# ryought/dbgphmm

Hardware: AMD Instinct MI355X
Metric: read-bases/sec through forward+backward P(R|X) (higher is better)
Workload: dtype f64; 1 GPU; cfg3: synthetic 100 kb diploid genome (1% divergence), 20x HiFi reads (p=0.001, L=1000), k=40 DBG; sparse-adaptive forward+backward+posteriors (generate_mappings); n_nodes=131694, n_edges=132357, reads_rank0=4026, bases_rank0=4000713, total_bases=4000713, spin_up_steps=12

## Files before the change

### dbgphmm_amd/csrc/api.cpp

```cpp
#include <chrono>
#include <cstdlib>
#include <cmath>
#include <cstring>

#include "phmm_internal.h"

namespace phmm {

static thread_local std::string g_error;
static thread_local hipStream_t g_stream = nullptr;
static thread_local uint64_t g_ws_limit = 0;
static thread_local CallStats g_stats;
static thread_local bool g_timing = false;

void set_error(const std::string &msg) { g_error = msg; }
int fail(int code, const std::string &msg) {
    g_error = msg;
    return code;
}
hipStream_t current_stream() { return g_stream; }
int &workset_index() {
    static thread_local int idx = 0;
    return idx;
}
ThreadContext capture_thread_context() {
    ThreadContext c{g_ws_limit, g_timing, 0};
    (void)hipGetDevice(&c.device);
    return c;
}
void adopt_thread_context(const ThreadContext &c, hipStream_t stream, int workset) {
    (void)hipSetDevice(c.device);
    g_ws_limit = c.ws_limit;
    g_timing = c.timing;
    g_stream = stream;
    g_stats = CallStats();
    workset_index() = workset;
}
static thread_local ShareInfo g_share;
CallStats &stats() { return g_stats; }
ShareInfo &share_info() { return g_share; }
bool timing_enabled() { return g_timing; }

uint64_t workspace_limit() {
    if (g_ws_limit) return g_ws_limit;
    size_t fr = 0, tot = 0;
    if (hipMemGetInfo(&fr, &tot) != hipSuccess) return (uint64_t)16 << 30;
    return (uint64_t)(0.8 * (double)fr);
}

static Knobs g_knobs;
const Knobs &knobs() { return g_knobs; }
void refresh_knobs() {
    auto flag = [](const char *n) {
        const char *e = std::getenv(n);
        return e != nullptr && e[0] != '\0' && !(e[0] == '0' && e[1] == '\0');
    };
    auto num = [](const char *n, int dflt) {
        const char *e = std::getenv(n);
        return e ? std::atoi(e) : dflt;
    };
    Knobs k;
    k.trace = flag("PHMM_TRACE");
    k.no_lean = flag("PHMM_NO_LEAN");
    k.no_wide_class = flag("PHMM_NO_WIDE_CLASS");
    k.no_packed = flag("PHMM_NO_PACKED");
    k.packed_cpl = num("PHMM_PACKED_CPL", 0);
    k.no_exact_hinted = flag("PHMM_NO_EXACT_HINTED");
    k.no_exact_dense = flag("PHMM_NO_EXACT_DENSE");
    k.no_wide_hinted = flag("PHMM_NO_WIDE_HINTED");
    k.wide_hinted = flag("PHMM_WIDE_HINTED") && !k.no_wide_hinted;
    k.no_wide_list_bwd = flag("PHMM_NO_WIDE_LIST_BWD");
    k.wide_edge_bwd = flag("PHMM_WIDE_EDGE_BWD");
    k.wide_states_bwd = flag("PHMM_WIDE_STATES_BWD");
    k.wide_bwd_t = num("PHMM_WIDE_BWD_T", 0);
    if (k.wide_bwd_t != 128 && k.wide_bwd_t != 448) k.wide_bwd_t = 0;
    k.wide_hinted_cpb = num("PHMM_WIDE_HINTED_CPB", 0);
    if (k.wide_hinted_cpb != 1 && k.wide_hinted_cpb != 2 && k.wide_hinted_cpb != 4) k.wide_hinted_cpb = 0;
    k.no_side_worker = flag("PHMM_NO_SIDE_WORKER");
    k.no_wide_handover = flag("PHMM_NO_WIDE_HANDOVER");
    k.workers = std::max(1, std::min(MAX_WORKERS, num("PHMM_WORKERS", 1)));
    k.warm_cols = num("PHMM_WARM_COLS", 0);
    k.chunk_groups = std::max(0, num("PHMM_CHUNK_GROUPS", 0));
    k.no_keep_all = flag("PHMM_NO_KEEP_ALL");
    k.pipeline_min_groups = std::max(1, num("PHMM_PIPELINE_MIN_GROUPS", 8));
    k.no_runmax = flag("PHMM_NO_RUNMAX");
    k.force_radix = flag("PHMM_FORCE_RADIX");
    k.no_bwd_skip = flag("PHMM_NO_BWD_SKIP");
    k.serial_emit = flag("PHMM_SERIAL_EMIT");
    k.emit_high_priority = flag("PHMM_EMIT_HIGH_PRIORITY");
    k.no_dma = flag("PHMM_NO_DMA");
    k.bwd_dma = flag("PHMM_BWD_DMA");
    k.dense_streams = num("PHMM_DENSE_STREAMS", 0);
    k.dense_w = num("PHMM_DENSE_W", 0);
    k.dense_npt = num("PHMM_DENSE_NPT", 0);
    if (const char *e = std::getenv("PHMM_MEM_FRACTION")) k.mem_fraction = std::min(0.97, std::max(0.1, std::atof(e)));
    k.share_prefix = num("PHMM_SHARE_PREFIX", -1);
    if (k.share_prefix < 0 || k.share_prefix > 6) k.share_prefix = -1;
    g_knobs = k;
}

void trace(const char *tag) {
    if (!g_knobs.trace) return;
    static thread_local std::chrono::steady_clock::time_point last = std::chrono::steady_clock::now();
    (void)hipStreamSynchronize(g_stream);
    const auto now = std::chrono::steady_clock::now();
    static const auto t0 = std::chrono::steady_clock::now();
    std::fprintf(stderr, "[phmm trace] w%d @%9.2f %-28s %8.2f ms\n", workset_index(),
                 std::chrono::duration<double, std::milli>(now - t0).count(), tag,
                 std::chrono::duration<double, std::milli>(now - last).count());
    last = now;
}

uint64_t table_budget(const DevicePool &pool, uint64_t reserve) {
    if (g_ws_limit) return g_ws_limit;
    size_t fr = 0, tot = 0;
    if (hipMemGetInfo(&fr, &tot) != hipSuccess) return (uint64_t)16 << 30;
    const double frac = g_knobs.mem_fraction > 0.0 ? g_knobs.mem_fraction : 0.9;
    const double b = frac * (double)(fr + pool.owned_table_bytes()) - (double)reserve;
    return (uint64_t)std::max(b, 64.0 * 1024 * 1024);
}
uint64_t planned_budget(const DevicePool &pool) {
    if (g_ws_limit) return g_ws_limit;
    size_t fr = 0, tot = 0;
    if (hipMemGetInfo(&fr, &tot) != hipSuccess) return (uint64_t)16 << 30;
    const double frac = g_knobs.mem_fraction > 0.0 ? g_knobs.mem_fraction : 0.95;
    return (uint64_t)(frac * (double)(fr + pool.owned_bytes()));
}

static std::mutex g_pool_mu;
static DevicePool *g_pools[64] = {};
DevicePool &device_pool() {
    int dev = 0;
    (void)hipGetDevice(&dev);
    if (dev < 0 || dev >= 64) PHMM_THROW(PHMM_ENODEVICE, "device index out of range");
    std::lock_guard<std::mutex> lk(g_pool_mu);
    if (!g_pools[dev]) {
        g_pools[dev] = new DevicePool();
        g_pools[dev]->device = dev;
    }
    return *g_pools[dev];
}
void DevicePool::recycle(DevBuf &b) {
    if (!b.p) return;
    std::lock_guard<std::mutex> lk(spare_mu);
    if (b.bytes < ((size_t)1 << 20) || b.bytes > SPARE_BYTES) {
        b.release();
        return;
    }
    while (!spare.empty() && (spare.size() >= SPARE_MAX || spare_total + b.bytes > SPARE_BYTES)) {
        (void)hipFree(spare.front().first);
        spare_total -= spare.front().second;
        spare.erase(spare.begin());
    }
    spare_total += b.bytes;
    const size_t n = b.bytes;
    spare.emplace_back(b.detach(), n);
}
void DevicePool::take(DevBuf &b, size_t n) {
    if (n <= b.bytes) return;
    {
        std::lock_guard<std::mutex> lk(spare_mu);
        int best = -1;
        for (int i = 0; i < (int)spare.size(); i++)
            if (spare[i].second >= n && spare[i].second <= 2 * n &&
                (best < 0 || spare[i].second < spare[best].second))
                best = i;
        if (best >= 0) {
            b.adopt(spare[best].first, spare[best].second);
            spare_total -= spare[best].second;
            spare.erase(spare.begin() + best);
// ... 892 lines not shown
```

### dbgphmm_amd/csrc/dense.hip

```cpp
#include <algorithm>
#include <cmath>
#include <cstring>
#include <numeric>
#include <type_traits>

#include "dense_internal.h"
#include "lds_dma.h"
#include "prefix_share.h"

#ifndef PHMM_FWD_PF
#define PHMM_FWD_PF 2
#endif
#ifndef PHMM_BWD_PF
#define PHMM_BWD_PF 1
#endif
#ifndef PHMM_SMALLW_WAVES
#define PHMM_SMALLW_WAVES 3
#endif

namespace phmm {


__device__ __forceinline__ int xcd_block(int b, int nblk8) {
    int per = nblk8 >> 3;
// ... 352 lines not shown
}

template <int W>
__global__ void __launch_bounds__(BLOCK) fwd_finish(const DenseArgs a) {
    __shared__ double lds[(BLOCK / 64) * 64];
    const int g = blockIdx.x;
    const int col = blockIdx.y;
    constexpr int ROWS = BLOCK / W;
    const int r = threadIdx.x % W, row = threadIdx.x / W;
    const int len = a.len[g * W + r];
    const size_t ecols = a.eall ? (size_t)a.Lc : 1;
    double s = 0.0;
    const bool live = a.eall ? col < len : len > 0;
    if (live)
        for (int b = row; b < a.nblk; b += ROWS)
            s += a.epart[(((size_t)g * ecols + col) * a.nblk8 + b) * W + r];
    const double tot = block_reduce_rows<W>(s, OpAdd(), lds);
    if (threadIdx.x < W && live) {
        const int E = a.FE[((size_t)g * (a.Lc + 1) + (a.eall ? col + 1 : len)) * W + r];
        const double lp = log(a.lp.p_end * tot) + (double)E * LN2;
        if (a.eall) a.logE[((size_t)g * a.Lc + col) * W + r] = lp;
        if (!a.eall || col == len - 1) a.logPf[g * W + r] = lp;
    }
}

__device__ __forceinline__ double dev_logadd(double x, double y) {
    const double hi = x >= y ? x : y, lo = x >= y ? y : x;
    if (lo == -INFINITY) return hi;
    return hi + log1p(exp(lo - hi));
}

template <int W>
__device__ __forceinline__ void bwd_chain(const DenseArgs &a, int g, int p, double *lds) {
    constexpr int ROWS = BLOCK / W;
    const int r = threadIdx.x % W, row = threadIdx.x / W;
    const int len = a.len[g * W + r];
    const bool live = p < len && (!a.bstart || p <= (a.bstart[g * W + r] & ~(1 << 30)));
    double s1 = 0.0, s2 = 0.0;
    if (live) {
        const double *bp = a.bpart + ((size_t)(p & 1) * a.ng + g) * a.nblk8 * W * 2;
        for (int b = row; b < a.nblk; b += ROWS) {
            s1 += bp[((size_t)b * W + r) * 2 + 0];
            s2 += bp[((size_t)b * W + r) * 2 + 1];
        }
    }
    const double t1 = block_reduce_rows<W>(s1, OpAdd(), lds);
    const double t2 = block_reduce_rows<W>(s2, OpAdd(), lds);
    if (threadIdx.x < W && live) {
        const size_t ix = ((size_t)g * (a.Lc + 1) + p) * W + r;
        const double E = (double)a.BE[ix] * LN2;
        const double ibn = (p + 1 < len) ? a.logibB[ix + W] : -INFINITY;
        const double lr = log(a.lp.p_random);
        a.logmbB[ix] = dev_logadd(log(t1) + E, log(a.lp.p_MI) + lr + ibn);
        a.logibB[ix] = dev_logadd(log(t2) + E, log(a.lp.p_II) + lr + ibn);
    }
}

static constexpr int BDMA_DEPTH = 3;
static constexpr int BDMA_SLOT = 5 * 64;
template <int W, bool DMA, bool VF = false>
__global__ void __launch_bounds__(BLOCK, (W == 64 ? 4 : PHMM_SMALLW_WAVES)) bwd_step(const DenseArgs a, const int pos) {
    static_assert(!VF || (W == 64 && !DMA), "the virtual-table loads go through the register ring of bwd_step<64>");
    __shared__ double lds[(BLOCK / 64) * 64];
    constexpr bool DMA_ = DMA && W == 64;
    __shared__ double ring[DMA_ ? (BLOCK / 64) * BDMA_DEPTH * BDMA_SLOT : 1];
    const int g = blockIdx.y + a.g_off;
    const int lb = xcd_block(blockIdx.x, a.nblk8);
    constexpr int ROWS = BLOCK / W;
    const int r = threadIdx.x % W;
    const int row = threadIdx.x / W;
    const int len = a.len[g * W + r];
    const int braw = a.bstart ? a.bstart[g * W + r] : len - 1;
    const bool sparse_tail = (braw & (1 << 30)) != 0;
    const int bstart = braw & ~(1 << 30);
    const bool live = pos < len && pos <= bstart;
    const bool first = live && pos == len - 1;
    const LinParams &lp = a.lp;
    const size_t NW = (size_t)a.N * W;

    if (lb == 0 && pos + 1 < a.Lc) bwd_chain<W>(a, g, pos + 1, lds);

    bool compute = true;
    int hull_first = 0, hull_top = a.npt - 1;
    if (W == 64 && a.skA) {
        compute = false;
        const int rho = __builtin_amdgcn_readfirstlane(lb * ROWS + row);
        if (__any(live) && rho < a.nrun) {
            const size_t gs = (size_t)g * a.nseg, gr = (size_t)g * a.nrun, par = (size_t)a.ng * a.nrun;
            const uint32_t *hh = a.skH + gs;
            const uint8_t *an = a.skA + (size_t)((pos + 1) & 1) * par + gr;
            const int sh = pos + 1 < 31 ? pos + 1 : 31;
            const int sprs = segs_per_run_log2(a.npt), spr = 1 << sprs;
            const unsigned anyfirst = __any(first) ? 1u : 0u;
            const int ls = threadIdx.x & 63;
            const int sg = rho * spr + ls;
            unsigned f = 0;
            if (ls < spr && sg < a.nseg) {
                f = (hh[sg] >> sh) | (((unsigned)an[rho] >> ls) & 1u) | anyfirst;
                const uint32_t o0 = a.rs_off[sg], o1 = a.rs_off[sg + 1];
                for (uint32_t q = o0; q < o1 && !f; q++) {
                    const uint32_t t = a.rs[q];
                    f = (hh[t] >> sh) | (((unsigned)an[t >> sprs] >> (t & (uint32_t)(spr - 1))) & 1u);
                }
            }
            const unsigned mask = (unsigned)__builtin_amdgcn_readfirstlane((int)(unsigned)__ballot(f != 0));
            const int kb = rho * a.npt;
            compute = seg_hull(mask, a.sseg, a.npt - 1 < a.N - 1 - kb ? a.npt - 1 : a.N - 1 - kb, &hull_first, &hull_top);
            if (ls == 0) a.skA[(size_t)(pos & 1) * par + gr + rho] = (uint8_t)mask;
        }
    }
    if (!__syncthreads_or(live && (compute || lb == 0))) {
        if (threadIdx.x < W && lb < a.nblk) {
            double *bp = a.bpart + ((size_t)(pos & 1) * a.ng + g) * a.nblk8 * W * 2;
            bp[((size_t)lb * W + r) * 2 + 0] = 0.0;
            bp[((size_t)lb * W + r) * 2 + 1] = 0.0;
        }
        if (a.want_map && a.Prun) a.Prun[((size_t)g * a.nblk8 + lb) * BLOCK + threadIdx.x] = 0.0;
        return;
    }

    int Epos = 0;
    double sc = 1.0;
    if (live && !first) {
        const unsigned long long cm = a.cmaxB[((size_t)g * a.Lc + (pos + 1)) * W + r];
        const int e = exp_of_bits(cm);
        sc = pow2(-e);
        Epos = a.BE[((size_t)g * (a.Lc + 1) + (pos + 1)) * W + r] + e;
    }
    const uint8_t x = live ? a.bases[((size_t)g * a.Lc + pos) * W + r] : (uint8_t)0;
    const int cn = a.bcols == 2 ? ((pos + 1) & 1) : (pos + 1 < a.Lc ? pos + 1 : 0);
    const int cc = a.bcols == 2 ? (pos & 1) : pos;
    const double *nm = a.Bm + ((size_t)g * a.bcols + cn) * NW;
    const double *ni = a.Bi + ((size_t)g * a.bcols + cn) * NW;
    double *om = a.Bm + ((size_t)g * a.bcols + cc) * NW;
    double *oi = a.Bi + ((size_t)g * a.bcols + cc) * NW;
    double *od = a.Bd ? a.Bd + ((size_t)g * a.bcols + cc) * NW : nullptr;

    double wgt = 0.0, wgt2 = 0.0;
    const double *fm = nullptr, *fi = nullptr, *fd = nullptr, *gm = nullptr, *gi = nullptr, *gd = nullptr;
    const bool want_post = a.want_freq || a.want_map;
    if (want_post && live) {
        const double lpf = a.logPf[g * W + r];
        if (lpf > -INFINITY) {
            if (pos >= 1) {
                const int fe = a.FE[((size_t)g * (a.Lc + 1) + (pos - 1)) * W + r];
                wgt = exp((double)(fe + Epos) * LN2 - lpf);
            }
            if (first && !sparse_tail) {
                const int fe = a.FE[((size_t)g * (a.Lc + 1) + pos) * W + r];
                wgt2 = exp((double)fe * LN2 - lpf) * lp.p_end;
            }
        }
    }
    if (want_post) {
        const size_t cprev = ((size_t)g * a.Lc + (pos > 0 ? pos - 1 : 0)) * NW;
        const size_t ccur = ((size_t)g * a.Lc + pos) * NW;
        fm = a.Fm + cprev; fi = a.Fi + cprev; fd = a.Fd + cprev;
        gm = a.Fm + ccur; gi = a.Fi + ccur; gd = a.Fd + ccur;
    }
    int rf = r;
    if (VF && want_post) {
        const uint32_t v = share_lane_of_column(a.vlane[g * W + r], pos - 1);
        const size_t vc = ((size_t)(v / SHARE_W) * a.vLc + (pos - 1)) * NW;
        fm = a.vFm + vc; fi = a.vFi + vc; fd = a.vFd + vc;
        rf = (int)(v % SHARE_W);
    }

    double vmax = 0.0, s1 = 0.0, s2 = 0.0, pmx = 0.0, pmx2 = 0.0;
    double *Pa = a.want_map ? a.Pa + (size_t)g * NW : nullptr;
    double *Pb = a.want_map ? a.Pb + (size_t)g * NW : nullptr;
    if (lb < a.nblk && compute) {
        constexpr int H = CHAIN_HOPS;
        const int kbase = lb * (a.npt * ROWS) + row * a.npt + hull_first;
        double E1 = 0.0, E2 = 0.0, E3 = 0.0, E4 = 0.0, E5 = 0.0, Q1 = 0.0, Q2 = 0.0, Q3 = 0.0, Q4 = 0.0, Q5 = 0.0, TE = 0.0;
        int nvalid = 0;
        constexpr int PFB = DMA_ ? BDMA_DEPTH : PHMM_BWD_PF;
        double nx_m[PFB], nx_i[PFB], nx_fm[PFB], nx_fi[PFB], nx_fd[PFB];
        const double *lfm = want_post ? fm : nm, *lfi = want_post ? fi : nm, *lfd = want_post ? fd : nm;
        const int jtop = hull_top < a.N - 1 - kbase ? hull_top : a.N - 1 - kbase;
        const int l64 = threadIdx.x & 63;
        const double *srcA = (l64 < 32 ? nm : ni) + 2 * (l64 & 31);
        const double *srcB = (l64 < 32 ? lfm : lfi) + 2 * (l64 & 31);
        const double *srcC = lfd + 2 * (l64 & 31);
        const uint32_t ring_base =
            DMA_ ? (uint32_t)__builtin_amdgcn_readfirstlane(
                       (int)(uint32_t)(uintptr_t)&ring[(threadIdx.x >> 6) * BDMA_DEPTH * BDMA_SLOT])
                 : 0u;
// ... 970 lines not shown
```

### dbgphmm_amd/csrc/dense_internal.h

```cpp
#pragma once

#include <vector>

#include "phmm_internal.h"
#include "seg_hull.h"

namespace phmm {

static constexpr double LN2 = 0.693147180559945309417232121458;
static constexpr int BLOCK = 256;

struct DenseArgs {
    int N, ng, Lc, nblk, npt;
    int g_off;
    const NodeRec *nodes;
    const uint8_t *emis;
    const double *init, *dinit, *tdinit;
    const uint32_t *fc_off;
    const FwdEntry *fc;
    const uint32_t *bc_off;
    const BwdEntry *bc;
    const uint32_t *fh_off, *bh_off;
    const HopEntry *fh, *bh;
    int hop_mode;
    LinParams lp;
    const double *logib;
    const uint8_t *bases;
    const int *len;
    double *Fm, *Fi, *Fd;
    int *FE;
    unsigned long long *cmaxF;
    double *epart;
    int eall;
    double *logPf;
    double *logE;
    double *Bm, *Bi, *Bd;
    int bcols;
    int *BE;
    unsigned long long *cmaxB;
    double *bpart;
    double *logmbB, *logibB;
    double *accg;
    int want_freq;
    int nblk8;
    unsigned long long *tmaxF;
    const int *bstart;
    int want_map;
    double *Pa, *Pb;
    double *Prun;
    unsigned long long *pmax;
    const int *wf_sw;
    const uint8_t *wf_mode;
    int *wf_sub;
    int *wf_cnt;
    uint32_t *wf_node;
    double *wf_tot;
    double wf_ratio;
    double wf_ub_a, wf_ub_b;
    const uint32_t *rs_off = nullptr, *rs = nullptr;
    uint32_t *skH = nullptr;
    uint8_t *skA = nullptr;
    int nrun = 0, nseg = 0, sseg = 1;
    unsigned long long *skcells = nullptr;
    const double *vFm = nullptr, *vFi = nullptr, *vFd = nullptr;
    const uint32_t *vlane = nullptr;
    int vLc = 0, vJ = 0;
};
static constexpr int WF_CAP = 1024;


struct Plan {
    int W, ng_total, npt, nblk, nblk8;
    std::vector<uint32_t> order;
};

Plan make_plan(const phmm_model *m, const phmm_reads *reads, int forced_w);
Plan make_plan_ids(const phmm_model *m, const phmm_reads *reads, const std::vector<uint32_t> &ids);
void layout(DenseArgs &a, int W, bool full_b, void *tables, void *misc, size_t &tb, size_t &mb,
            bool backward_only = false);
void fill_model_args(DenseArgs &a, const phmm_model *m);
void host_logib(const phmm_model *m, size_t n, std::vector<double> &out);
void launch_fwd_step(int W, const DenseArgs &a, int pos);
void launch_fwd_finish(int W, const DenseArgs &a);
void launch_bwd_step(int W, const DenseArgs &a, int pos);
void launch_bwd_finish(int W, const DenseArgs &a);

struct ExactTables {
    double *f_m, *f_i, *f_d, *f_scal, *b_m, *b_i, *b_d, *b_scal;
};
void exact_dense_reads(phmm_model *m, const uint8_t *bases, const uint64_t *off, const std::vector<uint32_t> &ids, double *lf,
                       double *lb, double *freq_dev, const ExactTables *tabs, double *edge_freq_dev = nullptr,
                       double *init_freq_dev = nullptr);
bool certify_dense(int N, int len, double log2P, const int *FE, const double *log2maxF, const int *BE, const double *log2maxB,
                   double log2_p_end);
bool certify_dense_cells(int N, int len, const int *E, const double *log2max, bool backward);

}
```

### dbgphmm_amd/csrc/mapping_flow.hip

```cpp
#include <algorithm>
#include <cmath>
#include <cstring>
#include <memory>

#include <hipcub/hipcub.hpp>

#include "sparse_dyn.h"
#include "lean_bwd_kernel.h"
#include "wide_bwd_kernel.h"

namespace phmm {

static constexpr int KMAX = PHMM_MAX_ACTIVE_NODES;

template <int CAP> struct FRec {
    double m[CAP], i[CAP], d[CAP];
    uint32_t id[CAP];
    int n, na, E;
};

template <int CAP> __device__ bool load_record(const RecPool &p, uint64_t pos_index, FRec<CAP> &f) {
    const uint64_t o1 = p.off[pos_index];
    if (o1 == 0) return false;
    const uint8_t *rec = p.base + (o1 - 8);
// ... 821 lines not shown
            const double u = bval[q];
            rank += (u > v) || (u == v && bid[q] < id);
        }
        if (rank < need && nabove + rank < KMAX) {
            ids[nabove + rank] = id;
            val[nabove + rank] = v;
        }
    }
    __syncthreads();
    const int tot = nabove + (nb < need ? nb : need);
    return tot < KMAX ? tot : KMAX;
}

__global__ void __launch_bounds__(BLOCK) emit_dense_map(const DenseMapArgs ma, const int pos, const int lanes) {
    __shared__ uint32_t ids[KMAX];
    __shared__ double val[KMAX];
    __shared__ uint16_t order[KMAX];
    const DenseArgs &a = ma.d;
    if ((int)blockIdx.x >= ma.wl_count[1]) return;
    const uint32_t item = ma.wl_big[blockIdx.x];
    const int gi = (int)(item % (uint32_t)lanes), which = (int)(item / (uint32_t)lanes);
    const int len = a.len[gi];
    if (len == 0) return;
    const int braw = a.bstart[gi];
    const bool sparse_tail = (braw & (1 << 30)) != 0;
    const int bstart = braw & ~(1 << 30);
    const bool live = pos < len && pos <= bstart;
    const bool mine = which == 0 ? (live && pos >= 1) : (live && pos == len - 1 && !sparse_tail);
    if (!mine) return;
    int *cnt = which == 0 ? ma.cntA : ma.cntB;
    const int c = cnt[gi];
    const int g = gi / ma.W, r = gi % ma.W;
    const int mi = which == 0 ? pos : len;
    int n = c < KMAX ? c : KMAX;
    if (c > KMAX) {
        const double *P = (which == 0 ? a.Pa : a.Pb) + (size_t)g * a.N * ma.W + r;
        const double vmax = __longlong_as_double((long long)a.pmax[((size_t)g * (a.Lc + 1) + mi) * ma.W + r]);
        n = block_top_from_column(P, ma.W, a.N, vmax * ma.ratio_lin, vmax, ids, val, ma.force_radix != 0);
    } else {
        const uint32_t *cn = (which == 0 ? ma.candA_node : ma.candB_node) + (size_t)gi * KMAX;
        const double *cv = (which == 0 ? ma.candA_val : ma.candB_val) + (size_t)gi * KMAX;
        for (int j = threadIdx.x; j < n; j += BLOCK) {
            ids[j] = cn[j];
            val[j] = cv[j];
        }
    }
    __syncthreads();
    if (ma.topk > 0 && n < ma.topk && n < a.N && threadIdx.x == 0) {
        const int want = ma.topk < a.N ? ma.topk : a.N;
        const int n0 = n;
        for (uint32_t k = 0; n < want && k < (uint32_t)a.N; k++) {
            bool present = false;
            for (int j = 0; j < n0; j++) present |= ids[j] == k;
            if (!present) {
                ids[n] = k;
                val[n] = 0.0;
                n++;
            }
        }
        cnt[gi] = -n;
    }
    __syncthreads();
    if (cnt[gi] < 0) n = -cnt[gi];
    __syncthreads();
    if (threadIdx.x >= 64) return;
    const uint64_t pidx = ma.lane_pos0[gi] + (uint64_t)(mi - 1);
    if (!emit_mapping<KMAX>(ma.mpool, pidx, ids, val, n, ma.ratio_lin, true, order, ma.topk,
                            (long long)ma.eoff[item])) {
        if (threadIdx.x == 0) atomicOr(&ma.err[gi], SP_ERR_POOL);
    }
    if (threadIdx.x == 0) cnt[gi] = 0;
}

__global__ void __launch_bounds__(BLOCK) gather_logb(const double *logmbB, int Lc, int W, int lanes, double *out) {
    const int gi = blockIdx.x * BLOCK + threadIdx.x;
    if (gi < lanes) out[gi] = logmbB[(size_t)(gi / W) * (Lc + 1) * W + gi % W];
}

__global__ void __launch_bounds__(BLOCK) merge_logp(const uint32_t *lanes, int n, const double *src, double *dst) {
    const int j = blockIdx.x * BLOCK + threadIdx.x;
    if (j < n) dst[lanes[j]] = src[lanes[j]];
}

namespace {
template <int W> void launch_post_collect(const DenseMapArgs &ma, int pos) {
    hipLaunchKernelGGL(post_collect<W>, dim3(ma.d.nblk, ma.d.ng), dim3(BLOCK), 0, current_stream(), ma, pos);
}
void launch_post_collect_w(int W, const DenseMapArgs &ma, int pos) {
    switch (W) {
    case 1: launch_post_collect<1>(ma, pos); break;
    case 2: launch_post_collect<2>(ma, pos); break;
    case 4: launch_post_collect<4>(ma, pos); break;
    case 8: launch_post_collect<8>(ma, pos); break;
    case 16: launch_post_collect<16>(ma, pos); break;
    case 32: launch_post_collect<32>(ma, pos); break;
    case 64: launch_post_collect<64>(ma, pos); break;
    default: PHMM_THROW(PHMM_EINTERNAL, "bad read-group width");
    }
}
}

void mapping_backward_chunk(MapChunk &mc, const std::vector<uint32_t> &sparse_lanes, MappingSink *sink,
                            const Plan &plan, int g0, uint64_t R) {
    hipStream_t s = current_stream();
    CallStats &st = stats();
    phmm_model *m = mc.m;
    const int W = mc.W, lanes = mc.lanes;
    const std::vector<int> &hl = *mc.hl, &hsw = *mc.hsw;
    const std::vector<uint64_t> &lp0 = *mc.lane_pos0;
    const size_t NW = (size_t)m->N * W;

    std::vector<int> hb(lanes, 0);
    std::vector<uint64_t> gp0(lanes + 1, 0);
    int pos_max = -1;
    for (int gi = 0; gi < lanes; gi++) {
        const size_t slot = (size_t)g0 * W + gi;
        if (hl[gi] == 0 || slot >= R) {
            hb[gi] = -1;
            continue;
        }
        gp0[gi] = sink->reads->off[plan.order[slot]];
        if (hsw[gi] < hl[gi]) hb[gi] = hsw[gi] | (1 << 30);
        else hb[gi] = hl[gi] - 1;
        pos_max = std::max(pos_max, hb[gi] & ~(1 << 30));
    }
    DevBuf &ctl = m->wset().aux[3], &pbuf = m->wset().aux[4];
    const bool skip = W == 64 && !knobs().no_bwd_skip && pos_max >= 0;
    const int sseg = seg_size(mc.a.npt);
    const RunSucc *rsucc = skip ? &model_run_successors(m, sseg) : nullptr;
    const size_t sk_nrun = ((size_t)m->N + mc.a.npt - 1) / mc.a.npt;
    size_t cb = 0;
    auto carve = [&](size_t bytes) {
        cb = (cb + 255) / 256 * 256;
        size_t o = cb;
        cb += bytes;
        return o;
    };
    const size_t o_bs = carve(sizeof(int) * lanes), o_ca = carve(sizeof(int) * lanes * 2), o_cb = carve(sizeof(int) * lanes * 2),
                 o_err = carve(sizeof(uint32_t) * lanes), o_cells = carve(sizeof(unsigned long long)), o_lanes = carve(sizeof(uint32_t) * std::max<size_t>(sparse_lanes.size(), 1)),
                 o_lp0 = carve(sizeof(uint64_t) * (lanes + 1)), o_gp0 = carve(sizeof(uint64_t) * (lanes + 1)),
                 o_stop = carve(sizeof(int) * lanes),
                 o_skh = carve(skip ? sizeof(uint32_t) * (size_t)mc.a.ng * rsucc->nseg : 0), o_ska = carve(skip ? 2 * (size_t)mc.a.ng * sk_nrun : 0),
                 o_bn = carve(sizeof(uint32_t) * (size_t)lanes * KMAX * 2), o_bv = carve(sizeof(double) * (size_t)lanes * KMAX * 2),
                 o_an = carve(sizeof(uint32_t) * (size_t)lanes * KMAX * 2), o_av = carve(sizeof(double) * (size_t)lanes * KMAX * 2),
                 o_hand = carve(sizeof(BHandoff) * (size_t)lanes), o_eoff = carve(sizeof(unsigned long long) * 2 * (size_t)lanes),
                 o_wls = carve(sizeof(uint32_t) * 2 * (size_t)lanes), o_wlb = carve(sizeof(uint32_t) * 2 * (size_t)lanes),
                 o_wlc = carve(sizeof(int) * 2), o_lb = carve(sizeof(double) * (size_t)lanes);
    ctl.reserve(cb);
    char *cp = (char *)ctl.p;
    const size_t prun_n = (size_t)mc.ngc * mc.a.nblk8 * BLOCK;
    bool need_pb = false;
    for (int gi = 0; gi < lanes; gi++) need_pb |= hb[gi] >= 0 && !(hb[gi] & (1 << 30));
    pbuf.reserve(((need_pb ? 3 : 2) * (size_t)mc.ngc * NW + prun_n) * sizeof(double));
    unsigned long long top_before = 0;
    HIP_CHECK(hipMemcpyAsync(&top_before, sink->mp.top, sizeof(top_before), hipMemcpyDeviceToHost, s));
    HIP_CHECK(hipStreamSynchronize(s));

    for (int attempt = 0;; attempt++) {
        HIP_CHECK(hipMemsetAsync(cp, 0, o_bn, s));
        HIP_CHECK(hipMemcpyAsync(cp + o_bs, hb.data(), sizeof(int) * lanes, hipMemcpyHostToDevice, s));
        HIP_CHECK(hipMemcpyAsync(cp + o_lp0, lp0.data(), sizeof(uint64_t) * (lanes + 1), hipMemcpyHostToDevice, s));
        HIP_CHECK(hipMemcpyAsync(cp + o_gp0, gp0.data(), sizeof(uint64_t) * (lanes + 1), hipMemcpyHostToDevice, s));
        if (!sparse_lanes.empty())
            HIP_CHECK(hipMemcpyAsync(cp + o_lanes, sparse_lanes.data(), sizeof(uint32_t) * sparse_lanes.size(),
                                     hipMemcpyHostToDevice, s));
        const RecPool mp = sink->mp;

        DenseArgs a = mc.a;
        a.want_freq = 0;
        a.want_map = 1;
        a.bstart = (const int *)(cp + o_bs);
        a.Pa = pbuf.as<double>();
        a.Pb = need_pb ? pbuf.as<double>() + 2 * (size_t)mc.ngc * NW : pbuf.as<double>();
        a.Prun = knobs().no_runmax ? nullptr : pbuf.as<double>() + (need_pb ? 3 : 2) * (size_t)mc.ngc * NW;
        const bool st_on = W == 64 && mc.main_plan;
        if (skip) {
            a.rs_off = rsucc->off.as<uint32_t>();
            a.rs = rsucc->ent.as<uint32_t>();
            a.nseg = (int)rsucc->nseg;
            a.sseg = sseg;
            a.nrun = (int)sk_nrun;
            a.skH = (uint32_t *)(cp + o_skh);
            a.skA = (uint8_t *)(cp + o_ska);
            a.skcells = st_on ? (unsigned long long *)(cp + o_cells) : nullptr;
            HIP_CHECK(hipMemsetAsync(pbuf.p, 0, sizeof(double) * 2 * (size_t)mc.ngc * NW, s));
        }
        HIP_CHECK(hipMemsetAsync(a.cmaxB, 0, sizeof(unsigned long long) * (size_t)a.ng * a.Lc * W, s));
        HIP_CHECK(hipMemsetAsync(a.pmax, 0, sizeof(unsigned long long) * (size_t)a.ng * (a.Lc + 1) * W, s));
        HIP_CHECK(hipMemsetAsync(a.BE, 0, sizeof(int) * (size_t)a.ng * (a.Lc + 1) * W, s));
        HIP_CHECK(hipMemsetAsync(a.Bm, 0, sizeof(double) * (size_t)a.ng * a.bcols * NW, s));
        HIP_CHECK(hipMemsetAsync(a.Bi, 0, sizeof(double) * (size_t)a.ng * a.bcols * NW, s));

        if (!sparse_lanes.empty()) {
            hipLaunchKernelGGL(merge_logp, dim3((unsigned)((sparse_lanes.size() + BLOCK - 1) / BLOCK)), dim3(BLOCK), 0, s,
                               (const uint32_t *)(cp + o_lanes), (int)sparse_lanes.size(), mc.d_logp_sparse, a.logPf);
            SparseBwdArgs ba{};
            ba.M = mc.fa_M;
            ba.d = a;
            ba.W = W;
            ba.Lb = mc.Lfull;
            ba.sw = mc.d_sw;
            ba.bases = mc.d_bases_full;
            ba.fpool = mc.fpool;
            ba.mpool = mp;
            ba.lane_pos0 = (const uint64_t *)(cp + o_lp0);
            ba.map_pos0 = (const uint64_t *)(cp + o_gp0);
            ba.lanes = (const uint32_t *)(cp + o_lanes);
            ba.ratio_lin = mc.ratio_lin;
            ba.topk = mc.topk;
            ba.err = (uint32_t *)(cp + o_err);
            ba.stop = (int *)(cp + o_stop);
            ba.hand = (BHandoff *)(cp + o_hand);
            std::vector<uint32_t> todo;
            std::vector<int> hstop(lanes);
            std::vector<uint32_t> herr2(lanes);
            const bool lean_ok =
                mc.topk == 0 && m->dev.max_degree <= (uint32_t)ADJ_DEG && !knobs().no_lean;
            const bool wide_ok = lean_ok && !knobs().no_wide_class;
            const int slice = mc.Lfull > 6144 ? 4096 : 0;
            std::vector<uint32_t> cont = sparse_lanes, big, fresh;
            bool first = true, any_err = false;
            int bursts = 0;
            auto launch = [&](int kind, int mode, int steps, const std::vector<uint32_t> &who) {
                HIP_CHECK(hipMemcpyAsync(cp + o_lanes, who.data(), sizeof(uint32_t) * who.size(), hipMemcpyHostToDevice, s));
                ba.mode = mode;
                ba.max_steps = steps;
                if (kind == 0 && lean_ok)
                    hipLaunchKernelGGL(lean_backward_kernel, dim3((unsigned)who.size()), dim3(64), 0, s, ba);
                else if (kind == 0)
                    hipLaunchKernelGGL((sparse_backward_kernel<64>), dim3((unsigned)who.size()), dim3(64), 0, s, ba);
                else if (wide_ok)
                    hipLaunchKernelGGL(wide_backward_kernel<false>, dim3((unsigned)who.size()), dim3(WBK_T), 0, s, ba);
                else
                    hipLaunchKernelGGL((sparse_backward_kernel<KMAX>), dim3((unsigned)who.size()), dim3(64), 0, s, ba);
                HIP_CHECK(hipGetLastError());
                st.launches[3]++;
                HIP_CHECK(hipMemcpyAsync(hstop.data(), ba.stop, sizeof(int) * lanes, hipMemcpyDeviceToHost, s));
                HIP_CHECK(hipMemcpyAsync(herr2.data(), ba.err, sizeof(uint32_t) * lanes, hipMemcpyDeviceToHost, s));
                HIP_CHECK(hipStreamSynchronize(s));
            };
            for (int turn = 0; turn < 100000 && !any_err && (!cont.empty() || !big.empty() || !fresh.empty()); turn++) {
                std::vector<uint32_t> ncont;
                if (!cont.empty()) {
                    launch(0, first ? 0 : 1, lean_ok ? slice : 0, cont);
                    for (uint32_t gi : cont) {
                        if (herr2[gi] & ~SP_STOP_SLICE) any_err = true;
                        else if (hstop[gi] == hsw[gi]) continue;
                        else if (herr2[gi] & SP_STOP_SLICE) ncont.push_back(gi);
                        else if (first && hstop[gi] == hl[gi]) fresh.push_back(gi);
                        else big.push_back(gi);
                    }
                    first = false;
                }
                if (any_err) break;
                const int burst = slice > 0 ? (64 << std::min(bursts, 5)) : 0;
                for (int pass = 0; pass < 2 && !any_err; pass++) {
                    std::vector<uint32_t> &who = pass == 0 ? fresh : big;
                    if (who.empty()) continue;
                    launch(1, pass == 0 ? 0 : 1, burst, who);
                    for (uint32_t gi : who) {
                        if (herr2[gi] & ~SP_STOP_SLICE) any_err = true;
                        else if (hstop[gi] != hsw[gi]) ncont.push_back(gi);
                    }
                    who.clear();
                    bursts++;
                }
                cont.swap(ncont);
            }
            todo = cont;
            todo.insert(todo.end(), big.begin(), big.end());
            todo.insert(todo.end(), fresh.begin(), fresh.end());
            if (!todo.empty()) {
                bool perr = false;
                HIP_CHECK(hipMemcpy(herr2.data(), ba.err, sizeof(uint32_t) * lanes, hipMemcpyDeviceToHost));
                for (uint32_t gi : sparse_lanes) perr |= (herr2[gi] & ~SP_STOP_SLICE) != 0;
                if (!perr) PHMM_THROW(PHMM_EINTERNAL, "sparse backward did not finish");
            }
        }
        trace("  sparse backward");
        DenseMapArgs ma{};
        ma.d = a;
        ma.W = W;
        ma.mpool = mp;
        ma.lane_pos0 = (const uint64_t *)(cp + o_gp0);
        ma.ratio_lin = mc.ratio_lin;
        ma.topk = mc.topk;
        ma.err = (uint32_t *)(cp + o_err);
        ma.eoff = (unsigned long long *)(cp + o_eoff);
        ma.wl_small = (uint32_t *)(cp + o_wls);
        ma.wl_big = (uint32_t *)(cp + o_wlb);
        ma.wl_count = (int *)(cp + o_wlc);
        std::vector<int> live_at((size_t)pos_max + 2, 0);
        for (int gi = 0; gi < lanes; gi++)
            if (hb[gi] >= 0) live_at[(size_t)(hb[gi] & ~(1 << 30))]++;
        for (int p = pos_max - 1; p >= 0; p--) live_at[(size_t)p] += live_at[(size_t)p + 1];
        ma.force_radix = knobs().force_radix ? 1 : 0;
        LaunchTimer lt(timing_enabled() && st_on);
        std::unique_lock<std::mutex> dense_lock;
        if (mc.dense_token) dense_lock = std::unique_lock<std::mutex>(*mc.dense_token);
        const int wi = workset_index();
        if (!m->pool->cstream[wi]) {
            int least = 0, greatest = 0;
            HIP_CHECK(hipDeviceGetStreamPriorityRange(&least, &greatest));
            HIP_CHECK(hipStreamCreateWithPriority(&m->pool->cstream[wi], hipStreamNonBlocking, knobs().emit_high_priority ? greatest : least));
        }
        for (auto &e : m->pool->cevent[wi])
            if (!e) HIP_CHECK(hipEventCreateWithFlags(&e, hipEventDisableTiming));
        hipStream_t s2 = knobs().serial_emit ? s : m->pool->cstream[wi];
        hipEvent_t *ev_col = &m->pool->cevent[wi][0], *ev_emit = &m->pool->cevent[wi][2];
        bool emitted[2] = {false, false};
        for (int pos = pos_max; pos >= 0; pos--) {
            const int par = pos & 1;
            a.Pa = pbuf.as<double>() + (size_t)par * mc.ngc * NW;
            ma.d = a;
            ma.cntA = (int *)(cp + o_ca) + (size_t)par * lanes;
            ma.cntB = (int *)(cp + o_cb) + (size_t)par * lanes;
            ma.candA_node = (uint32_t *)(cp + o_an) + (size_t)par * lanes * KMAX;
            ma.candA_val = (double *)(cp + o_av) + (size_t)par * lanes * KMAX;
            ma.candB_node = (uint32_t *)(cp + o_bn) + (size_t)par * lanes * KMAX;
            ma.candB_val = (double *)(cp + o_bv) + (size_t)par * lanes * KMAX;
            if (emitted[par]) HIP_CHECK(hipStreamWaitEvent(s, ev_emit[par], 0));
            lt.begin();
            launch_bwd_step(W, a, pos);
            lt.end();
            launch_post_collect_w(W, ma, pos);
            HIP_CHECK(hipEventRecord(ev_col[par], s));
            HIP_CHECK(hipStreamWaitEvent(s2, ev_col[par], 0));
            hipLaunchKernelGGL(emit_offsets, dim3(1), dim3(1024), 0, s2, ma, pos, lanes);
            {
                const int ub = std::max(1, live_at[(size_t)pos] * (need_pb ? 2 : 1));
                hipLaunchKernelGGL(emit_dense_small, dim3((unsigned)std::min(1024, (ub + BLOCK / 64 - 1) / (BLOCK / 64))), dim3(BLOCK), 0,
                                   s2, ma, pos, lanes);
                hipLaunchKernelGGL(emit_dense_map, dim3((unsigned)ub), dim3(BLOCK), 0, s2, ma, pos, lanes);
            }
            HIP_CHECK(hipEventRecord(ev_emit[par], s2));
            emitted[par] = true;
            if (st_on) st.launches[1]++;
        }
        for (int par = 0; par < 2; par++)
            if (emitted[par]) HIP_CHECK(hipStreamWaitEvent(s, ev_emit[par], 0));
        HIP_CHECK(hipGetLastError());
        const bool want_lb = mc.logb_out && pos_max >= 0 && lanes > 0;
        if (want_lb) {
            launch_bwd_finish(W, a);
            hipLaunchKernelGGL(gather_logb, dim3((unsigned)((lanes + BLOCK - 1) / BLOCK)), dim3(BLOCK), 0, s, (const double *)a.logmbB,
                               a.Lc, W, lanes, (double *)(cp + o_lb));
            HIP_CHECK(hipGetLastError());
        }
        st.ms[1] += lt.total_ms();
        for (int gi = 0; gi < lanes; gi++)
            if (st_on && !a.skcells && hb[gi] >= 0) st.cells[1] += (uint64_t)((hb[gi] & ~(1 << 30)) + 1) * m->N;
        const size_t err_words = (o_cells + sizeof(unsigned long long) - o_err) / sizeof(uint32_t);
        std::vector<uint32_t> herr(err_words);
        HIP_CHECK(hipMemcpyAsync(herr.data(), cp + o_err, sizeof(uint32_t) * err_words, hipMemcpyDeviceToHost, s));
        if (want_lb) HIP_CHECK(hipMemcpyAsync(mc.logb_out, cp + o_lb, sizeof(double) * lanes, hipMemcpyDeviceToHost, s));
        HIP_CHECK(hipStreamSynchronize(s));
        if (a.skcells) {
            unsigned long long nc = 0;
            memcpy(&nc, herr.data() + (o_cells - o_err) / sizeof(uint32_t), sizeof nc);
            st.cells[1] += nc;
        }
        if (dense_lock.owns_lock()) dense_lock.unlock();
// ... 828 lines not shown
```

### dbgphmm_amd/csrc/phmm_internal.h

```cpp
#pragma once

#include <hip/hip_runtime.h>

#include <cstdint>
#include <cstdio>
#include <memory>
#include <mutex>
#include <string>
#include <vector>

#include "../../include/phmm_amd.h"
#include "../../include/phmm_amd_states.h"
#include "../../include/phmm_amd_path.h"
#include "../../include/phmm_amd_share.h"
#include "../../include/phmm_amd_sample.h"
#include "../../include/phmm_amd_generate.h"

namespace phmm {

void set_error(const std::string &msg);
int fail(int code, const std::string &msg);

struct Error {
    int code;
// ... 262 lines not shown
    std::vector<uint32_t> g_of;
    std::vector<uint32_t> g_cn;
    std::vector<uint32_t> g_emit;
    std::vector<uint32_t> g_seen;
    std::vector<uint32_t> g_at;
    uint32_t g_stamp = 0;
    phmm::DevBuf d_g_off, d_g_nodes, d_g_slot, d_bp_off, d_bp_slot;
};

namespace phmm {

struct CallStats {
    double ms[5] = {0, 0, 0, 0, 0};
    uint64_t launches[5] = {0, 0, 0, 0, 0};
    uint64_t cells[5] = {0, 0, 0, 0, 0};
};
CallStats &stats();
bool timing_enabled();
struct ShareInfo {
    int J = 0;
    uint64_t lanes = 0;
};
ShareInfo &share_info();

struct LaunchTimer {
    bool on;
    std::vector<hipEvent_t> ev;
    explicit LaunchTimer(bool on_) : on(on_) {}
    ~LaunchTimer() {
        for (auto e : ev) (void)hipEventDestroy(e);
    }
    void begin() {
        if (!on) return;
        hipEvent_t e;
        HIP_CHECK(hipEventCreate(&e));
        HIP_CHECK(hipEventRecord(e, current_stream()));
        ev.push_back(e);
    }
    void end() { begin(); }
    double total_ms() {
        if (!on || ev.empty()) return 0.0;
        HIP_CHECK(hipEventSynchronize(ev.back()));
        double t = 0.0;
        for (size_t k = 0; k + 1 < ev.size(); k += 2) {
            float ms = 0;
            HIP_CHECK(hipEventElapsedTime(&ms, ev[k], ev[k + 1]));
            t += ms;
        }
        return t;
    }
};

void trace(const char *tag);

struct Knobs {
    bool trace = false;
    bool no_lean = false;
    bool no_wide_class = false;
    bool no_packed = false;
    int packed_cpl = 0;
    bool no_exact_hinted = false;
    bool no_exact_dense = false;
    bool wide_hinted = false;
    bool no_wide_hinted = false;
    bool no_wide_list_bwd = false;
    bool wide_edge_bwd = false;
    bool wide_states_bwd = false;
    int wide_bwd_t = 0;
    int wide_hinted_cpb = 0;
    bool no_side_worker = false;
    bool no_wide_handover = false;
    int workers = 1;
    int warm_cols = 0;
    int chunk_groups = 0;
    bool no_keep_all = false;
    int pipeline_min_groups = 8;
    bool no_runmax = false;
    bool force_radix = false;
    bool serial_emit = false;
    bool emit_high_priority = false;
    bool no_dma = false;
    bool bwd_dma = false;
    bool no_bwd_skip = false;
    int dense_streams = 0;
    int dense_w = 0;
    int dense_npt = 0;
    double mem_fraction = 0.0;
    int share_prefix = -1;
};
const Knobs &knobs();
void refresh_knobs();

void model_build_host(phmm_model *m);
void model_upload(phmm_model *m);
const RunSucc &model_run_successors(phmm_model *m, int seg);

void run_dense(phmm_model *m, const phmm_reads *reads, double *out_lf, double *out_lb,
               double *out_nf);
void full_prob_sparse_backward(phmm_model *m, const phmm_reads *reads, double *out_logp, double *out_total);
void backward_sparse_tables(phmm_model *m, const uint8_t *read, uint64_t len, double *b_m, double *b_i, double *b_d,
                            double *b_scal, uint8_t *is_dense);
void run_sparse(phmm_model *m, const phmm_reads *reads, double *out_lf, double *out_lb, double *out_nf);
void run_dense_edges(phmm_model *m, const phmm_reads *reads, double *out_lf, double *out_ef, double *out_if);
struct RecPool;
void full_prob_reads_hinted(phmm_model *m, const phmm_reads *reads, const phmm_mappings *mp, uint32_t n_cand,
                            const double *init_logp, const double *trans_logp, double *out_logp,
                            double *out_total, const RecPool *pool = nullptr, const uint32_t *copy_nums = nullptr,
                            uint32_t min_copy_num = 0);
void full_prob_reads_copy_num_changes(phmm_model *m, const phmm_reads *reads, const phmm_mappings *mp,
                                      const uint32_t *base_cn, uint32_t min_cn, uint32_t n_cand, const uint64_t *chg_off,
                                      const uint32_t *chg_node, const uint32_t *chg_cn, double *out_logp,
                                      double *out_total, uint64_t *out_n_rescored);
void likelihood_refresh(phmm_likelihood *lk);
void likelihood_score_changes(phmm_likelihood *lk, uint32_t n_cand, const uint64_t *chg_off, const uint32_t *chg_node,
                              const uint32_t *chg_cn, double *out_logp, double *out_total, uint64_t *out_n_rescored,
                              bool by_group = false);
void likelihood_move(phmm_likelihood *lk, uint64_t n_chg, const uint32_t *chg_node, const uint32_t *chg_cn,
                     double *out_total, uint64_t *out_n_rescored, bool by_group = false);
void likelihood_current(const phmm_likelihood *lk, uint32_t *out_cn, double *out_logp, double *out_total);
void upload_reads(const phmm_reads *r);
void upload_mappings(const phmm_mappings *mp);
void mappings_map_nodes(phmm_model *m, const phmm_reads *reads, const phmm_mappings *mp_in, const uint32_t *map_off,
                        const uint32_t *map_nodes, uint32_t n_old, phmm_mappings **out);
void generate_mappings_hinted(phmm_model *m, const phmm_reads *reads, const phmm_mappings *mp_in, int use_max_ratio,
                              phmm_mappings **out, double *out_node_freq);
void run_with_mapping_edges(phmm_model *m, const phmm_reads *reads, const phmm_mappings *mp_in, double *out_lf,
                            double *out_ef, double *out_if);
void run_with_mapping_states(phmm_model *m, const phmm_reads *reads, const phmm_mappings *mp_in, double *out_lf,
                             double *out_state_logp, uint32_t *out_best);
void run_with_mapping_best_path(phmm_model *m, const phmm_reads *reads, const phmm_mappings *mp, double *out_logp,
                                uint32_t *out_path, uint32_t *out_counts);
void run_with_mapping_sample_paths(phmm_model *m, const phmm_reads *reads, const phmm_mappings *mp, uint32_t n_samples,
                                   uint64_t seed, double *out_logp, double *out_path_logp, uint32_t *out_path,
                                   uint32_t *out_counts, uint32_t *out_node_usage);
void sample_reads(phmm_model *m, uint64_t first_index, uint64_t n_walks, uint32_t length, uint32_t length_kind,
                  const uint32_t *start_nodes, uint64_t n_start_nodes, uint64_t seed, uint8_t *out_bases, uint32_t *out_len,
                  uint32_t *out_flags, uint32_t *out_history, uint32_t history_cap, uint32_t *out_history_len,
                  uint32_t *out_node_usage);
struct MappingSink;
void full_prob_reads_sparse(phmm_model *m, const phmm_reads *reads, double *out_logp, double *out_total,
                            MappingSink *sink, bool by_ratio = true, double *out_logb = nullptr);
void generate_mappings_sparse(phmm_model *m, const phmm_reads *reads, phmm_mappings **out, double *out_node_freq,
                              bool by_ratio = true);
void ensure_logib(phmm_model *m, size_t len);
void put_doubles(double *dst, const double *src_host, size_t n);
void put_bytes(void *dst, const void *src_host, size_t n);
void dense_tables(phmm_model *m, const uint8_t *read, uint64_t len, double *f_m, double *f_i,
                  double *f_d, double *f_scal, double *b_m, double *b_i, double *b_d,
                  double *b_scal);

}
```

### dbgphmm_amd/csrc/seg_hull.h

```cpp
#pragma once

#if defined(__HIPCC__)
#define PHMM_SEG_FN __host__ __device__ inline
#else
#define PHMM_SEG_FN inline
#endif

namespace phmm {

static constexpr int SEGS_PER_RUN = 8;

PHMM_SEG_FN int seg_size(int npt) { return npt % SEGS_PER_RUN == 0 ? npt / SEGS_PER_RUN : npt; }

static constexpr int SEGS_PER_RUN_LOG2 = 3;
static_assert(SEGS_PER_RUN == 1 << SEGS_PER_RUN_LOG2, "a run's byte of A holds one bit per segment");
PHMM_SEG_FN int segs_per_run_log2(int npt) { return npt % SEGS_PER_RUN == 0 ? SEGS_PER_RUN_LOG2 : 0; }

PHMM_SEG_FN bool seg_hull(unsigned mask, int S, int jtop, int *first, int *top) {
    if (!mask) return false;
    const int lo = __builtin_ctz(mask), hi = 31 - __builtin_clz(mask);
    const int t = hi * S + S - 1;
    *first = lo * S;
    *top = (t < jtop ? t : jtop) - lo * S;
    return true;
}

}
```

Measured before the change: 36.98 million bases/s.

## Precompute backward skip marks for all positions in a separate kernel pass

Result: no change. 36.73 million bases/s (-0.7%).

```diff
diff --git a/dbgphmm_amd/csrc/api.cpp b/dbgphmm_amd/csrc/api.cpp
--- a/dbgphmm_amd/csrc/api.cpp
+++ b/dbgphmm_amd/csrc/api.cpp
@@ -86,6 +86,7 @@
     k.no_runmax = flag("PHMM_NO_RUNMAX");
     k.force_radix = flag("PHMM_FORCE_RADIX");
     k.no_bwd_skip = flag("PHMM_NO_BWD_SKIP");
+    k.bwd_marks_inline = flag("PHMM_BWD_MARKS_INLINE");
     k.serial_emit = flag("PHMM_SERIAL_EMIT");
     k.emit_high_priority = flag("PHMM_EMIT_HIGH_PRIORITY");
     k.no_dma = flag("PHMM_NO_DMA");
diff --git a/dbgphmm_amd/csrc/dense.hip b/dbgphmm_amd/csrc/dense.hip
--- a/dbgphmm_amd/csrc/dense.hip
+++ b/dbgphmm_amd/csrc/dense.hip
@@ -458,7 +458,15 @@
 
     bool compute = true;
     int hull_first = 0, hull_top = a.npt - 1;
-    if (W == 64 && a.skA) {
+    if (W == 64 && a.skAll) {
+        compute = false;
+        const int rho = __builtin_amdgcn_readfirstlane(lb * ROWS + row);
+        if (rho < a.nrun) {
+            const unsigned mask = a.skAll[((size_t)pos * a.ng + g) * a.nrun + rho];
+            const int kb = rho * a.npt;
+            compute = seg_hull(mask, a.sseg, a.npt - 1 < a.N - 1 - kb ? a.npt - 1 : a.N - 1 - kb, &hull_first, &hull_top);
+        }
+    } else if (W == 64 && a.skA) {
         compute = false;
         const int rho = __builtin_amdgcn_readfirstlane(lb * ROWS + row);
         if (__any(live) && rho < a.nrun) {
@@ -471,14 +479,7 @@
             const int ls = threadIdx.x & 63;
             const int sg = rho * spr + ls;
             unsigned f = 0;
-            if (ls < spr && sg < a.nseg) {
-                f = (hh[sg] >> sh) | (((unsigned)an[rho] >> ls) & 1u) | anyfirst;
-                const uint32_t o0 = a.rs_off[sg], o1 = a.rs_off[sg + 1];
-                for (uint32_t q = o0; q < o1 && !f; q++) {
-                    const uint32_t t = a.rs[q];
-                    f = (hh[t] >> sh) | (((unsigned)an[t >> sprs] >> (t & (uint32_t)(spr - 1))) & 1u);
-                }
-            }
+            if (ls < spr && sg < a.nseg) f = seg_mark(hh, an, a.rs_off, a.rs, sg, sh, sprs, anyfirst);
             const unsigned mask = (unsigned)__builtin_amdgcn_readfirstlane((int)(unsigned)__ballot(f != 0));
             const int kb = rho * a.npt;
             compute = seg_hull(mask, a.sseg, a.npt - 1 < a.N - 1 - kb ? a.npt - 1 : a.N - 1 - kb, &hull_first, &hull_top);
diff --git a/dbgphmm_amd/csrc/dense_internal.h b/dbgphmm_amd/csrc/dense_internal.h
--- a/dbgphmm_amd/csrc/dense_internal.h
+++ b/dbgphmm_amd/csrc/dense_internal.h
@@ -60,6 +60,7 @@
     const uint32_t *rs_off = nullptr, *rs = nullptr;
     uint32_t *skH = nullptr;
     uint8_t *skA = nullptr;
+    const uint8_t *skAll = nullptr;
     int nrun = 0, nseg = 0, sseg = 1;
     unsigned long long *skcells = nullptr;
     const double *vFm = nullptr, *vFi = nullptr, *vFd = nullptr;
diff --git a/dbgphmm_amd/csrc/mapping_flow.hip b/dbgphmm_amd/csrc/mapping_flow.hip
--- a/dbgphmm_amd/csrc/mapping_flow.hip
+++ b/dbgphmm_amd/csrc/mapping_flow.hip
@@ -927,6 +927,30 @@
     if (j < n) dst[lanes[j]] = src[lanes[j]];
 }
 
+__global__ void __launch_bounds__(BLOCK) bwd_marks(const DenseArgs a, uint8_t *A_all, const int pos) {
+    const int g = blockIdx.y;
+    bool live = false, first = false;
+    if (threadIdx.x < 64) {
+        const int len = a.len[g * 64 + threadIdx.x];
+        const int bstart = a.bstart[g * 64 + threadIdx.x] & ~(1 << 30);
+        live = pos < len && pos <= bstart;
+        first = live && pos == len - 1;
+    }
+    const bool glive = __syncthreads_or(live) != 0;
+    const unsigned anyfirst = __syncthreads_or(first) ? 1u : 0u;
+    const int sprs = segs_per_run_log2(a.npt), spr = 1 << sprs;
+    const int sg = blockIdx.x * BLOCK + threadIdx.x;
+    const int rho = sg >> sprs, ls = sg & (spr - 1);
+    const size_t par = (size_t)a.ng * a.nrun, gr = (size_t)g * a.nrun;
+    unsigned f = 0;
+    if (glive && sg < a.nseg)
+        f = seg_mark(a.skH + (size_t)g * a.nseg, A_all + (size_t)(pos + 1) * par + gr, a.rs_off, a.rs, sg,
+                     pos + 1 < 31 ? pos + 1 : 31, sprs, anyfirst);
+    const unsigned long long bal = __ballot(f != 0);
+    const unsigned mask = spr == 1 ? (f != 0 ? 1u : 0u) : (unsigned)(bal >> (threadIdx.x & 63 & ~(SEGS_PER_RUN - 1))) & 0xffu;
+    if (ls == 0 && rho < a.nrun) A_all[(size_t)pos * par + gr + rho] = (uint8_t)mask;
+}
+
 namespace {
 template <int W> void launch_post_collect(const DenseMapArgs &ma, int pos) {
     hipLaunchKernelGGL(post_collect<W>, dim3(ma.d.nblk, ma.d.ng), dim3(BLOCK), 0, current_stream(), ma, pos);
@@ -986,6 +1010,7 @@
                  o_lp0 = carve(sizeof(uint64_t) * (lanes + 1)), o_gp0 = carve(sizeof(uint64_t) * (lanes + 1)),
                  o_stop = carve(sizeof(int) * lanes),
                  o_skh = carve(skip ? sizeof(uint32_t) * (size_t)mc.a.ng * rsucc->nseg : 0), o_ska = carve(skip ? 2 * (size_t)mc.a.ng * sk_nrun : 0),
+                 o_aall = carve(skip ? (size_t)(pos_max + 2) * mc.a.ng * sk_nrun : 0),
                  o_bn = carve(sizeof(uint32_t) * (size_t)lanes * KMAX * 2), o_bv = carve(sizeof(double) * (size_t)lanes * KMAX * 2),
                  o_an = carve(sizeof(uint32_t) * (size_t)lanes * KMAX * 2), o_av = carve(sizeof(double) * (size_t)lanes * KMAX * 2),
                  o_hand = carve(sizeof(BHandoff) * (size_t)lanes), o_eoff = carve(sizeof(unsigned long long) * 2 * (size_t)lanes),
@@ -1028,6 +1053,7 @@
             a.skH = (uint32_t *)(cp + o_skh);
             a.skA = (uint8_t *)(cp + o_ska);
             a.skcells = st_on ? (unsigned long long *)(cp + o_cells) : nullptr;
+            a.skAll = knobs().bwd_marks_inline ? nullptr : (const uint8_t *)(cp + o_aall);
             HIP_CHECK(hipMemsetAsync(pbuf.p, 0, sizeof(double) * 2 * (size_t)mc.ngc * NW, s));
         }
         HIP_CHECK(hipMemsetAsync(a.cmaxB, 0, sizeof(unsigned long long) * (size_t)a.ng * a.Lc * W, s));
@@ -1123,6 +1149,13 @@
             }
         }
         trace("  sparse backward");
+        if (a.skAll) {
+            const int spr = 1 << segs_per_run_log2(a.npt);
+            const dim3 mgrid((unsigned)((sk_nrun * spr + BLOCK - 1) / BLOCK), (unsigned)a.ng);
+            for (int pos = pos_max; pos >= 0; pos--)
+                hipLaunchKernelGGL(bwd_marks, mgrid, dim3(BLOCK), 0, s, a, (uint8_t *)(cp + o_aall), pos);
+            HIP_CHECK(hipGetLastError());
+        }
         DenseMapArgs ma{};
         ma.d = a;
         ma.W = W;
diff --git a/dbgphmm_amd/csrc/phmm_internal.h b/dbgphmm_amd/csrc/phmm_internal.h
--- a/dbgphmm_amd/csrc/phmm_internal.h
+++ b/dbgphmm_amd/csrc/phmm_internal.h
@@ -368,6 +368,7 @@
     bool no_dma = false;
     bool bwd_dma = false;
     bool no_bwd_skip = false;
+    bool bwd_marks_inline = false;
     int dense_streams = 0;
     int dense_w = 0;
     int dense_npt = 0;
diff --git a/dbgphmm_amd/csrc/seg_hull.h b/dbgphmm_amd/csrc/seg_hull.h
--- a/dbgphmm_amd/csrc/seg_hull.h
+++ b/dbgphmm_amd/csrc/seg_hull.h
@@ -16,6 +16,18 @@
 static_assert(SEGS_PER_RUN == 1 << SEGS_PER_RUN_LOG2, "a run's byte of A holds one bit per segment");
 PHMM_SEG_FN int segs_per_run_log2(int npt) { return npt % SEGS_PER_RUN == 0 ? SEGS_PER_RUN_LOG2 : 0; }
 
+PHMM_SEG_FN unsigned seg_mark(const unsigned *hh, const unsigned char *an, const unsigned *rs_off, const unsigned *rs, int sg,
+                              int sh, int sprs, unsigned anyfirst) {
+    const unsigned low = (1u << sprs) - 1u;
+    unsigned f = (hh[sg] >> sh) | (((unsigned)an[sg >> sprs] >> ((unsigned)sg & low)) & 1u) | anyfirst;
+    const unsigned o0 = rs_off[sg], o1 = rs_off[sg + 1];
+    for (unsigned q = o0; q < o1 && !f; q++) {
+        const unsigned t = rs[q];
+        f = (hh[t] >> sh) | (((unsigned)an[t >> sprs] >> (t & low)) & 1u);
+    }
+    return f;
+}
+
 PHMM_SEG_FN bool seg_hull(unsigned mask, int S, int jtop, int *first, int *top) {
     if (!mask) return false;
     const int lo = __builtin_ctz(mask), hi = 31 - __builtin_clz(mask);
```
